# watsonyanghx/GAN_Lib_Tensorflow

Measured on AMD Instinct MI355X. Metric: images/sec (G+D step) SNGAN-ResNet CIFAR-10 bs=64, higher is better.
Workload: dtype bf16; 1 GPU; SNGAN ResNet CIFAR-10 32x32 bs=64 hinge: 1 G update (2x64 fakes) + 5 D updates (64 real + 64 fake) per step; global_batch=64, per_gpu_batch=64, parallelism=dp1, graphs=True, finite=True, collectives_in_graphs=False, grad_wire=fp32

## Files before the change

gan_lib_tensorflow_amd/SNGAN/gan_cifar_resnet.py:

```python
import contextlib
import math
import sys

import numpy as np
import torch
import torch.distributed as _dist

from .. import functional as Fn
from .. import graphs
from .. import kernels as K
from .. import parallel
from ..common import resnet_block as blocks
from ..common.ops import embedding as _embedding
from ..common.ops import linear as _linear
from ..common.ops import conv2d as _conv2d
from ..common.ops import normalization as _normalization
from ..common.ops import sn as _sn
from ..common.ops.sn import NO_OPS
from ..store import ParamStore, get_default_store, set_default_store

BATCH_SIZE = 64
GEN_BS_MULTIPLE = 2
ITERS = 100000
DIM_G = 128
# ... 75 lines not shown
        return 2
    if blocks.FUSE_RES8 and W.dim() == 4 and tuple(W.shape) == (3, 3, 128, 128) and ('D.Block.3.' in name or 'D.Block.4.' in name):
        return 4
    if Fn.IMG16_CONV and name.endswith('D.Block.2.Conv1/Filters') and W.dim() == 4 and W.shape[0] == 3 and W.shape[2] % 64 == 0 and W.shape[3] % 128 == 0 \
            and W.shape[2] % 128 == 0:
        if Fn.FACTOR_LABEL_CONV and LABEL_TABLE and CONDITIONAL and W.shape[2] == 2 * DIM_D:
            return 6
        return 4
    return 0


def _g_prep_kind(name, W):
    if Fn.RES8_CONV and name.endswith(('G.Block.1.Conv1/Filters', 'G.Block.1.Conv2/Filters')) and W.dim() == 4 and W.shape[0] == 3 \
            and W.shape[2] in (128, 256) and W.shape[3] % 128 == 0:
        return 4
    if Fn.PHASE_UPCONV and name.endswith('.Conv1/Filters') and W.dim() == 4 and W.shape[0] == 3:
        return 1
    if Fn.IMG16_CONV and name.endswith('G.Block.2.Conv2/Filters') and W.dim() == 4 and W.shape[0] == 3 and W.shape[2] % 128 == 0 and W.shape[3] % 128 == 0:
        return 4
    return 0


FUSE_SN_TAIL = True
FUSE_FEED = True
LABEL_TABLE = True
FUSED_HEAD = True
HEAD_IN_CHAIN = True


def Discriminator(inputs, labels, update_collection=None, reuse=False, loss_head=None):
# ... 656 lines not shown
```

gan_lib_tensorflow_amd/_lib.py:

```python
import ctypes as C
import os

_HERE = os.path.dirname(os.path.abspath(__file__))
DTYPE = os.environ.get("GANK_DTYPE", "bf16").lower()
if DTYPE not in ("bf16", "fp16"):
    raise RuntimeError(f"GANK_DTYPE={DTYPE!r}: bf16 or fp16")
ACT_DTYPE_NAME = "bfloat16" if DTYPE == "bf16" else "float16"
LIB_PATH = os.path.join(_HERE, os.environ.get("GANK_LIB_NAME", "libgank.so" if DTYPE == "bf16" else "libgank_f16.so"))

P, I, L, F = C.c_void_p, C.c_int, C.c_long, C.c_float

IN_UPSAMPLE2X, IN_RELU, OUT_TANH, DY_UPSAMPLE2X, RES_UPSAMPLE2X, STATS_PREZEROED, OUT_POOLSUM2X = 1, 2, 4, 8, 64, 256, 512
STAT_SLOTS = 16


class SnDesc(C.Structure):
    _fields_ = [(n, P) for n in ("W", "u_in", "u_out", "v", "W_bar", "scal", "a", "b", "bpart",
                                 "dW_bar", "dW", "rowdot", "ga", "u_snap")] + \
               [("K", I), ("C", I), ("row_offset", I), ("chunk_offset", I)]


class WgradItem(C.Structure):
    _fields_ = [("x", P), ("dy", P), ("dw", P), ("dbias", P)]

# ... 51 lines not shown
    "gank_conv2d_general_dgrad": [P, P, P, P, I, I, I, I, I, I, I, I, I, P],
    "gank_conv2d_general_wgrad": [P, P, P, P, I, I, I, I, I, I, I, I, I, I, I, P],
    "gank_res8_chain_fwd": [P, P, P, P, P, P, I, I, I, P],
    "gank_res8_chain_bwd": [P, P, P, P, P, P, P, P, P, I, I, I, P],
    "gank_phase_stack4": [P, P, I, I, I, P],
    "gank_pad_rows": [P, P, C.c_long, I, I, I, I, P],
    "gank_tile_rows": [P, P, I, I, I, P],
    "gank_fewout_pack": [P, P, I, I, I, I, I, P],
    "gank_zero_f32": [P, C.c_long, P],
    "gank_img16_conv3x3": [P, P, P, P, P, P, I, I, I, I, P],
    "gank_cbn_relu_img16_conv3x3": [P, P, P, P, P, P, P, P, P, I, I, I, I, I, I, P, I, P],
    "gank_img16_conv3x3_stats": [P, P, P, P, P, P, I, I, I, I, P, I, P],
    "gank_res8_chain_fwd_head": [P, P, P, P, P, P, P, P, P, I, I, I, P],
    "gank_res8_chain_bwd_head": [C.POINTER(Res8Head), P, P, P, P, P, P, P, I, I, I, P],
    "gank_res8_conv3x3": [P, P, P, P, P, I, I, I, I, P, I, P],
    "gank_im2col_narrow": [P, P, I, I, I, I, I, I, I, I, I, I, P],
    "gank_tap_gather_up2": [P, P, P, I, I, I, I, I, I, I, I, P],
    "gank_tap_scatter_up2": [P, P, I, I, I, I, I, I, I, P],
    "gank_depth_to_space2": [P, P, I, I, I, I, P],
    "gank_space_to_depth2": [P, P, I, I, I, I, P],
    "gank_cpool_res_fprop": [P, P, P, P, P, I, I, I, I, I, I, P],
    "gank_cpool_res_dgrad": [P, P, P, P, I, I, I, I, I, P],
    "gank_cpool_res_dgrad_image_wgrad": [P, P, P, P, P, P, P, P, P, I, I, I, I, I, P, P],
    "gank_sum_slabs": [C.POINTER(SlabJob), I, P],
    "gank_convpool3x3_wgrad_job": [P, P, P, P, P, L, I, I, I, I, I, I, C.POINTER(SlabJob), P],
    "gank_conv2d_wgrad_slab_elems": [I, I, I, I, I, I, I],
    "gank_conv2d_wgrad_slabs": [P, P, P, P, I, I, I, I, I, I, I, F, P, L, C.POINTER(SlabJob), P],
    "gank_conv2d_wgrad_slab_splits": [I, I, I, I, I, I, I],
    "gank_conv2d_wgrad_slabs_rows": [P, P, P, P, I, I, I, I, I, I, I, I, F, P, L, C.POINTER(SlabJob), P],
    "gank_conv2d_wgrad_slabs_rows_tap_sums": [P, P, P, P, I, I, I, I, I, I, I, I, F, P, L, C.POINTER(SlabJob), P, I, P, P],
# ... 158 lines not shown
```

gan_lib_tensorflow_amd/csrc/conv_resident.hip:

```cpp
#include "gank_common.h"
#include "label_conv_dev.h"
#ifdef GANK_TUNING
static __device__ int gank_stats_dbg = 0;
static void gank_stats_dbg_init() {
  static const int v = gank_tune("GANK_STATS_DBG", 0);
  static bool done = false;
  if (!done) { done = true; if (v) (void)hipMemcpyToSymbol(HIP_SYMBOL(gank_stats_dbg), &v, sizeof(int)); }
}
#else
static inline void gank_stats_dbg_init() {}
#endif
#include <stdlib.h>

namespace {
constexpr int RB_C = 128;
constexpr int RB_PPB = RB_C * 2 + 16;
constexpr int RB_RPB = 2944;
constexpr int RB_IMG = 10 * RB_RPB;
constexpr int RB_STEPS = 9 * (RB_C / 16);
constexpr int RB_WBYTES = RB_C * 9 * RB_C * 2;
constexpr int RB_LDS = 2 * RB_IMG;

struct ResFwdArgs {
  const bf16* x;
// ... 2121 lines not shown
  }
  const int grid = N * (Cout / 128);
  if (Cin == 256) {
    constexpr int LDS = G8Geom<256>::IMG > G8_RED_BYTES ? G8Geom<256>::IMG : G8_RED_BYTES;
    GANK_MAX_DYNAMIC_LDS((res8_conv3x3_kernel<256, 12>), LDS, "res8_conv3x3");
    hipLaunchKernelGGL((res8_conv3x3_kernel<256, 12>), dim3(grid), dim3(256), LDS, s, a);
  } else {
    constexpr int LDS = G8Geom<128>::IMG > G8_RED_BYTES ? G8Geom<128>::IMG : G8_RED_BYTES;
    GANK_MAX_DYNAMIC_LDS((res8_conv3x3_kernel<128, 12>), LDS, "res8_conv3x3");
    hipLaunchKernelGGL((res8_conv3x3_kernel<128, 12>), dim3(grid), dim3(256), LDS, s, a);
  }
  gank_prof_end(0, s);
  GANK_LAUNCH_OK("res8_conv3x3");
  return 0;
}
```

gan_lib_tensorflow_amd/csrc/prep_weights.h:

```cpp
#pragma once
#include "gank_common.h"

template <bool SC>
__device__ __forceinline__ float prep_ld(float x, float sg) {
  if constexpr (SC) return x / sg;
  else return x;
}

__device__ __forceinline__ void up_range_R(int a, int i, int& lo, int& hi) {
  if (a == 0) { lo = i == 0 ? 0 : 1; hi = i == 0 ? 0 : 2; } else { lo = i == 0 ? 0 : 2; hi = i == 0 ? 1 : 2; }
}
__device__ __forceinline__ void up_range_S(int u, int& lo, int& hi) {
  lo = u == 0 ? 2 : (u == 1 ? 1 : 0);
  hi = u == 0 ? 2 : (u == 1 ? 2 : (u == 2 ? 1 : 0));
}
template <bool SC = false>
__device__ __forceinline__ float sum_taps(const float* __restrict__ p, long plane, bool flip, int h0, int h1, int w0, int w1, float sg = 1.f) {
  const float mh = h1 > h0 ? 1.f : 0.f, mw = w1 > w0 ? 1.f : 0.f;
  const int t00 = flip ? (2 - h0) * 3 + (2 - w0) : h0 * 3 + w0, t01 = flip ? (2 - h0) * 3 + (2 - w1) : h0 * 3 + w1;
  const int t10 = flip ? (2 - h1) * 3 + (2 - w0) : h1 * 3 + w0, t11 = flip ? (2 - h1) * 3 + (2 - w1) : h1 * 3 + w1;
  const float a = prep_ld<SC>(p[t00 * plane], sg), b = prep_ld<SC>(p[t01 * plane], sg), c = prep_ld<SC>(p[t10 * plane], sg), d = prep_ld<SC>(p[t11 * plane], sg);
  return ((a + mw * b) + mh * c) + (mh * mw) * d;
}

// ... 182 lines not shown
      const int lane = (int)(q & 63);
      long u = q >> 6;
      const int kk = (int)(u % (kc / 16)); u /= (kc / 16);
      const int tap = (int)(u % taps);
      const int rt = (int)(u / taps);
      const int row = rt * 32 + (lane & 31), k0 = kk * 16 + (lane >> 5) * 8;
      bf16x8 o;
#pragma unroll
      for (int j = 0; j < 8; j++) {
        const int k = k0 + j;
        const long cp = d.cin_pitch > 0 ? d.cin_pitch : d.Cin;
        o[j] = f2bf(prep_ld<SC>(isf ? d.w[((long)tap * cp + k) * d.Cout + row] : d.w[((long)(taps - 1 - tap) * cp + row) * d.Cout + k], sg));
      }
      *reinterpret_cast<bf16x8*>(dst + q * 8) = o;
    }
  } else if (d.kind == 5) {
    const bool isf = b < t.nwf[e];
    const long q = (long)(isf ? b : b - t.nwf[e]) * 256 + threadIdx.x;
    const long nchunk = 2L * d.Cin * d.Cout;
    if (q < nchunk) {
      const int lane = (int)(q & 63), r = lane & 31, hh = lane >> 5;
      long u = q >> 6;
      bf16x8 o;
      if (isf) {
        const int kk = (int)(u & 3); u >>= 2;
        const int tap = (int)(u & 15); u >>= 4;
        const int nch = d.Cin >> 6;
        const int chunk = (int)(u % nch), co = (int)(u / nch) * 32 + r;
        int h0, h1, w0, w1;
        up_range_S(tap >> 2, h0, h1);
// ... 76 lines not shown
    }
  }
}


static inline int prep_table_fill(PrepTable& t, const gank_prep_desc* table, int count, int base_index) {
  t = PrepTable{};
  t.count = count;
  int blocks = 0;
  for (int i = 0; i < t.count; i++) {
    const gank_prep_desc& d = table[i];
    const bool ok = d.w && (d.wf || d.wd) && d.ksize >= 1 && d.Cin > 0 && d.Cout > 0;
    if (!ok) { gank_set_error("prep_weights_batched: bad entry %d", base_index + i); return -1; }
    const bool kind_ok = d.kind == 0 || ((d.kind == 1 || d.kind == 2) && d.ksize == 3 && d.wf && d.wd) ||
                         (d.kind == 4 && d.Cin % 32 == 0 && d.Cout % 32 == 0 && (d.cin_pitch == 0 || d.cin_pitch >= d.Cin)) ||
                         (d.kind == 5 && d.ksize == 3 && d.wf && d.wd && d.Cin % 64 == 0 && d.Cout % 32 == 0);
    if (!kind_ok) {
      gank_set_error("prep_weights_batched: entry %d: kind %d needs ksize 3 and both outputs (1, 2, 5) / channels %% 32 == 0 (4) / Cin %% 64 == 0 (5)", base_index + i, d.kind);
      return -1;
    }
    t.d[i] = d;
    const int taps = d.ksize * d.ksize;
    int nwf = d.wf ? (roundup(taps * d.Cin, 64) / 64) * (roundup(d.Cout, 32) / 32) : 0;
    int nwd = d.wd ? cdiv((long)roundup(d.Cin, 32) * roundup(taps * d.Cout, 64), 2048) : 0;
    if (d.kind == 1 || d.kind == 2) {
      t.up[i] = d.kind == 1 ? prep_up_args(1, d.w, d.wf, d.wd, d.Cin, d.Cout) : prep_up_args(2, d.w, d.wd, d.wf, d.Cin, d.Cout);
      const PrepUpSplit sp = prep_up_split(t.up[i], d.kind);
      nwf = sp.ntiles;
      nwd = sp.nelem;
    }
    if (d.kind == 5) nwf = nwd = cdiv(2L * d.Cin * d.Cout, 256);
    if (d.kind == 4) {
      nwf = d.wf ? cdiv((long)d.Cout * taps * d.Cin / 8, 256) : 0;
      nwd = d.wd ? cdiv((long)d.Cin * taps * d.Cout / 8, 256) : 0;
    }
    t.first_block[i] = blocks;
    t.nwf[i] = nwf;
    blocks += nwf + nwd;
  }
  t.first_block[t.count] = blocks;
  return blocks;
}
```

gan_lib_tensorflow_amd/functional.py:

```python
import torch
from torch.autograd import Function

from . import kernels as K

BF16 = K.BF16
POOL_CONV4 = True
CPOOL_RESIDENT = True
PHASE_UPCONV = True
RES8_CONV = True
UPCONV_WGRAD_PHASE = True
IMG16_CONV = True


_boundary_log = None


def boundary(x, tag):
    if _boundary_log is not None and x.requires_grad:
        _boundary_log.append((tag, x))
    return x


class record_boundaries:
    def __enter__(self):
        global _boundary_log
# ... 126 lines not shown
            k, cin, cout = 1, W.shape[0], W.shape[1]
        else:
            k, cin, cout = W.shape[0], W.shape[2], W.shape[3]
        assert x.dim() == 4 and x.shape[3] == cin, (tuple(x.shape), tuple(W.shape))
        assert not (pool_out and (out_tanh or upsample))
        n, h, w, _ = x.shape
        H, Wd = (2 * h, 2 * w) if upsample else (h, w)
        flags = (K.IN_UPSAMPLE2X if upsample else 0) | (K.IN_RELU if in_relu else 0) | (K.OUT_TANH if out_tanh else 0)
        b = bias.detach() if bias is not None else None
        res_up = residual is not None and getattr(residual, "_up2x", False)
        ctx.res_up_orig = res_up
        res8 = (RES8_CONV and k == 3 and not in_relu and not pool_out and not out_tanh and getattr(W, "_prep_res", None) is not None
                and K.res8_conv3x3_ok(n, (H, Wd), cin, cout))
        img16 = (IMG16_CONV and k == 3 and not upsample and not pool_out and not out_tanh
                 and getattr(W, "_prep_res", None) is not None and K.img16_conv3x3_ok(n, (H, Wd), cin, cout))
        phase = upsample and k == 3 and cin % 64 == 0 and not in_relu and PHASE_UPCONV and not res8
        pool4 = pool_out and k == 3 and cin % 64 == 0 and cout % 64 == 0 and POOL_CONV4
        if res_up and (phase or pool_out):
            residual = K.unpool2x2_add(residual, None, 1.0)
            res_up = False
        if res8:
            rflags = (K.IN_UPSAMPLE2X if upsample else 0) | (K.RES_UPSAMPLE2X if res_up else 0)
            if stats_groups:
                y, _Conv2d.last_stats = K.res8_conv3x3(x, W._prep_res[0], b, cout, rflags, residual, stats_groups)
            else:
                y = K.res8_conv3x3(x, W._prep_res[0], b, cout, rflags, residual)
        elif img16:
            iflags = (K.IN_RELU if in_relu else 0) | (K.RES_UPSAMPLE2X if res_up else 0)
            if stats_groups:
                y, _Conv2d.last_stats = K.img16_conv3x3(x, W._prep_res[0], b, cout, iflags, None, residual, stats_groups)
            else:
                y = K.img16_conv3x3(x, W._prep_res[0], b, cout, iflags, None, residual)
        elif phase:
            wph, _ = getattr(W, "_prep_up", None) or K.upconv3x3_prep(W.detach().view(3, 3, cin, cout))
            if stats_groups and not out_tanh:
                y, _Conv2d.last_stats = K.upconv3x3_fprop(x, wph, b, cout, 0, residual, stats_groups)
            else:
                y = K.upconv3x3_fprop(x, wph, b, cout, K.OUT_TANH if out_tanh else 0, residual)
        elif pool4 and getattr(W, "_prep_cpres", None) is not None:
            y = K.cpool_res_fprop(x, W._prep_cpres[0], b, cout, K.IN_RELU if in_relu else 0, residual)
        elif pool4:
            wp4, _ = getattr(W, "_prep_pool", None) or K.convpool3x3_prep(W.detach().view(3, 3, cin, cout))
            y = K.convpool3x3_fprop(x, wp4, b, cout, K.IN_RELU if in_relu else 0, residual)
        elif pool_out:
            wf, _ = _prepared(W, k, cin, cout, True, False)
            yfull = K.conv2d_fprop(x, wf, b, (H, Wd), cout, k, flags)
            y = K.pool2x2(yfull, 0.25, residual)
# ... 7 lines not shown
                if stats_groups and not out_tanh:
                    y, _Conv2d.last_stats = K.conv2d_fprop(x, wf, b, (H, Wd), cout, k, flags | (K.RES_UPSAMPLE2X if res_up else 0), 1.0, residual,
                                                           stats_groups=stats_groups)
                else:
                    y = K.conv2d_fprop(x, wf, b, (H, Wd), cout, k, flags | (K.RES_UPSAMPLE2X if res_up else 0), 1.0, residual)
        ctx.res_up = res_up
        ctx.add_link = ctx.res_link = None
        link = getattr(x, "_add_link", None)
        if link is not None and ctx.needs_input_grad[0] and not (upsample or pool_out or phase or pool4 or res8):
            link.armed = True
            ctx.add_link = link
        rlink = getattr(residual, "_grad_link", None) if residual is not None else None
        if rlink is not None and rlink.armed and not res_up and not ctx.res_up_orig:
            ctx.res_link = rlink
        ctx.save_for_backward(x, W, y if out_tanh else None)
        ctx.cfg = (k, cin, cout, H, Wd, upsample, in_relu, pool_out, out_tanh, bias, phase, pool4)
        if FUSE_IMAGE_WGRAD and x.is_cuda:
            if (k == 3 and cin == 3 and residual is None and not (upsample or in_relu or pool_out or out_tanh or stats_groups)
                    and ctx.needs_input_grad[1] and not ctx.needs_input_grad[0]):
                ctx.sink = _Conv2d.last_sink = ImageWgradSink(x, W, bias)
                ctx.set_materialize_grads(False)
            elif (pool4 and in_relu and getattr(W, "_prep_cpres", None) is not None and ctx.needs_input_grad[0]
                  and getattr(x, "_image_wgrad_sink", None) is not None and K.cpool_res_dgrad_image_wgrad_ok(y, cin)):
                ctx.isink = x._image_wgrad_sink
                ctx.ssink = getattr(residual, "_shortcut_sink", None) if (residual is not None and not ctx.res_up_orig) else None
        ctx.res8 = res8 and W._prep_res[1] is not None and K.res8_conv3x3_ok(n, (8, 8), cout, cin)
        ctx.img16 = img16 and W._prep_res[1] is not None and K.img16_conv3x3_ok(n, (16, 16), cout, cin)
        return y

    @staticmethod
    def backward(ctx, dy):
# ... 35 lines not shown
            elif (CONV1X1_BWD_ONE_LAUNCH and k == 1 and wflags == 0 and scale == 1.0 and ctx.needs_input_grad[0] and ctx.add_link is None
                  and not ctx.img16 and not ctx.res8 and not phase
                  and int(K.lib().gank_conv2d_wgrad_slab_elems(x.shape[0], H, Wd, cin, cout, 1, 0)) == 0
                  and K.conv1x1_wgrad_dgrad_ok(x.shape[0], (H, Wd), cin, cout, _prepared(W, k, cin, cout, False, True)[1])):
                dx_fused = K.conv1x1_wgrad_dgrad(x, g, tgt, _prepared(W, k, cin, cout, False, True)[1], dbias=btgt)
            else:
                K.conv2d_wgrad(x, g, tgt, (H, Wd), k, wflags, scale, dbias=btgt,
                               slab_jobs=_slab_jobs if (SLAB_WGRADS and BATCH_SMALL_WGRADS) else None)
            dW = None if acc else tgt
        elif btgt is not None:
            K.colsum(g, btgt, 1.0)
        if dx_fused is not None:
            dx = dx_fused
        elif ctx.needs_input_grad[0] and ctx.res8:
            dx = K.res8_conv3x3(g, W._prep_res[1], None, cin, K.OUT_POOLSUM2X if upsample else 0)
        elif ctx.needs_input_grad[0] and phase:
            prep = getattr(W, "_prep_up", None) or K.upconv3x3_prep(W.detach().view(3, 3, cin, cout))
            dx = K.upconv3x3_dgrad(g, prep[1], cin)
        elif ctx.needs_input_grad[0] and pool4 and getattr(W, "_prep_cpres", None) is not None and ctx.isink is not None:
            isink, ssink = ctx.isink, ctx.ssink
            t1, _, b1, _ = isink.targets()
            ts = bs_ = xp = None
            if ssink is not None:
                ts, _, bs_, _ = ssink.targets()
                xp = ssink.x
            K.cpool_res_dgrad_image_wgrad(g, W._prep_cpres[1], x, isink.x, t1, b1, xp, ts, bs_,
                                          slab_jobs=_slab_jobs if (SLAB_WGRADS and BATCH_SMALL_WGRADS) else None)
            isink.done = True
            if ssink is not None:
                ssink.done = True
# ... 409 lines not shown
        if self.opt is not None:
            self.opt.pending_sn = None
        return self

    def __exit__(self, *exc):
        global SN_DEFER_APPLY
        SN_DEFER_APPLY = self.prev
        return False


def spectral_norm_batch(Ws, us, snapshot=False, inplace=False, prep=None, label=None, state=None):
    batch = K.SnBatch(list(Ws), [u.detach() for u in us], snapshot, inplace, state=state)
    batch.prep, batch.label = prep, label
    outs = _SpectralNorm.apply(batch, *Ws)
    for o, wb in zip(outs, batch.W_bar):
        for attr in ("_prep", "_prep_up", "_prep_pool", "_prep_res", "_prep_cpres", "_label_T"):
            val = getattr(wb, attr, None)
            if val is not None and o is not wb:
                setattr(o, attr, val)
    return outs, batch


CBN_REMASK = True


class _CondBatchNorm(Function):
    @staticmethod
    def forward(ctx, x, labels, gamma, beta, groups, relu):
        cs = getattr(x, "_cbn_stats", None)
        if cs is not None and cs.groups == groups and cs.sums.shape[-1] == x.shape[-1]:
            y, stats = K.cbn_fwd_from_sums(x, labels, gamma.detach(), beta.detach(), cs, relu)
# ... 843 lines not shown
```

gan_lib_tensorflow_amd/kernels.py:

```python
import ctypes as C

import torch

from . import _lib
from ._lib import IN_UPSAMPLE2X, IN_RELU, OUT_TANH, DY_UPSAMPLE2X, RES_UPSAMPLE2X, STATS_PREZEROED, OUT_POOLSUM2X, SnDesc, PrepDesc, WgradItem, LabelDenseDesc, Res8Head, SlabJob

BF16, F32, I32 = getattr(torch, _lib.ACT_DTYPE_NAME), torch.float32, torch.int32


def _stream():
    return C.c_void_p(torch.cuda.current_stream().cuda_stream)


def _p(t, dtype=None, name="tensor"):
    if t is None:
        return None
    if not t.is_cuda:
        raise RuntimeError(f"gank: {name} must live on the GPU (no CPU path exists)")
    if not t.is_contiguous():
        raise RuntimeError(f"gank: {name} must be contiguous, got strides {t.stride()} for {tuple(t.shape)}")
    if dtype is not None and t.dtype != dtype:
        raise RuntimeError(f"gank: {name} must be {dtype}, got {t.dtype}")
    return C.c_void_p(t.data_ptr())

# ... 3 lines not shown


def lib():
    return _lib.load()


def prep_weights(w, want_f=True, want_d=False):
    k, _, cin, cout = w.shape
    taps = k * k
    wf = torch.empty((_roundup(cout, 32), _roundup(taps * cin, 64)), dtype=BF16, device=w.device) if want_f else None
    wd = torch.empty((_roundup(cin, 32), _roundup(taps * cout, 64)), dtype=BF16, device=w.device) if want_d else None
    _lib.check(lib().gank_conv2d_prep_weights(_p(w, F32, "w"), _p(wf), _p(wd), k, cin, cout, _stream()), "prep_weights")
    return wf, wd


_PREP_ATTR = ("_prep", "_prep_up", "_prep_pool", None, "_prep_res", "_prep_cpres", "_prep_feat")


def _prep_plan(ws, want_d=True, kinds=None, sources=None):
    kinds = list(kinds) if kinds is not None else [0] * len(ws)
    todo = [i for i, kd in enumerate(kinds) if kd is not None]
    table = (PrepDesc * max(len(todo), 1))()
    outs = []
    for slot, i in enumerate(todo):
        w, kind = ws[i], kinds[i]
        if w.dim() == 2:
            k, cin, cout = 1, w.shape[0], w.shape[1]
        else:
            k, cin, cout = w.shape[0], w.shape[2], w.shape[3]
        taps = k * k
        dev = w.device
# ... 13 lines not shown
            wf, wd = getattr(w, "_prep_pool", None) or (torch.empty((_roundup(cout, 32), _roundup(16 * cin, 64)), dtype=BF16, device=dev),
                                                       torch.empty((4, _roundup(cin, 32), 4 * cout), dtype=BF16, device=dev))
        elif kind == 4:
            assert k == 3 and cin % 32 == 0 and cout % 32 == 0
            wf, wd = getattr(w, "_prep_res", None) or (torch.empty(taps * cin * cout, dtype=BF16, device=dev),
                                                      torch.empty(taps * cin * cout, dtype=BF16, device=dev) if want_d else None)
        elif kind == 5:
            assert k == 3 and cin % 64 == 0 and cout % 32 == 0
            wf, wd = getattr(w, "_prep_cpres", None) or (torch.empty(16 * cin * cout, dtype=BF16, device=dev),
                                                        torch.empty(16 * cin * cout, dtype=BF16, device=dev))
        elif kind == 6:
            assert k == 3 and cin % 64 == 0 and cout % 32 == 0
            half = cin // 2
            wf, wd = getattr(w, "_prep_feat", None) or (torch.empty(taps * half * cout, dtype=BF16, device=dev),
                                                       torch.empty(taps * half * cout, dtype=BF16, device=dev) if want_d else None)
        else:
            raise ValueError(f"unknown preparation kind {kind}")
        src = w if sources is None else sources[i]
        d = table[slot]
        d.w, d.wf, d.wd = _p(src.detach(), F32, "w").value, wf.data_ptr(), (wd.data_ptr() if wd is not None else None)
        d.ksize, d.Cin, d.Cout, d.kind = k, cin, cout, kind
        if kind == 6:
            d.Cin, d.kind, d.cin_pitch = cin // 2, 4, cin
        outs.append((wf, wd))
    return table, todo, outs


def _prep_attach(ws, kinds, todo, outs):
    for i, o in zip(todo, outs):
        setattr(ws[i], _PREP_ATTR[kinds[i]], o)
# ... 464 lines not shown
    return y


def res8_conv3x3(x, rf, bias, cout, flags=0, residual=None, stats_groups=0):
    n, cin = x.shape[0], x.shape[3]
    hw = 4 if flags & OUT_POOLSUM2X else 8
    y = torch.empty((n, hw, hw, cout), dtype=BF16, device=x.device)
    if stats_groups:
        sums, pre = stats_arena.take((stats_groups, _lib.STAT_SLOTS, 2, cout), x.device)
        _lib.check(lib().gank_res8_conv3x3(_p(x, BF16, "x"), _p(rf, BF16, "rf"), _p(bias, F32, "bias"), _p(residual, BF16, "residual"), _p(y),
                                           n, cin, cout, flags | (STATS_PREZEROED if pre else 0), _p(sums), stats_groups, _stream()), "res8_conv3x3")
        return y, ConvStats(sums, bias, stats_groups)
    _lib.check(lib().gank_res8_conv3x3(_p(x, BF16, "x"), _p(rf, BF16, "rf"), _p(bias, F32, "bias"), _p(residual, BF16, "residual"), _p(y),
                                       n, cin, cout, flags, None, 0, _stream()), "res8_conv3x3")
    return y


def cpool_res_fprop(x, rf, bias, cout, flags=0, residual=None):
    n, h, w, cin = x.shape
    y = torch.empty((n, h // 2, w // 2, cout), dtype=BF16, device=x.device)
    _lib.check(lib().gank_cpool_res_fprop(_p(x, BF16, "x"), _p(rf, BF16, "rf"), _p(bias, F32, "bias"), _p(residual, BF16, "residual"),
                                          _p(y), n, h // 2, w // 2, cin, cout, flags, _stream()), "cpool_res_fprop")
    return y


def cpool_res_dgrad(dy, rd, cin, relu_ref=None):
    n, hp, wp, cout = dy.shape
    dx = torch.empty((n, 2 * hp, 2 * wp, cin), dtype=BF16, device=dy.device)
    _lib.check(lib().gank_cpool_res_dgrad(_p(dy, BF16, "dy"), _p(rd, BF16, "rd"), _p(relu_ref, BF16, "relu_ref"), _p(dx),
                                          n, hp, wp, cin, cout, _stream()), "cpool_res_dgrad")
# ... 1224 lines not shown
```

include/gank.h:

```cpp
#ifndef GANK_H
#define GANK_H

#include <stddef.h>
#include <stdint.h>

#ifdef __cplusplus
extern "C" {
#endif

#define GANK_VERSION 100

#define GANK_IN_UPSAMPLE2X 1
#define GANK_IN_RELU 2
#define GANK_OUT_TANH 4
#define GANK_DY_UPSAMPLE2X 8
#define GANK_STAT_SLOTS 16
#define GANK_STATS_PREZEROED 256
#define GANK_RES_UPSAMPLE2X 64
#define GANK_OUT_POOLSUM2X 512

int gank_version(void);
int gank_act_dtype(void);
const char* gank_last_error(void);

// ... 84 lines not shown
                             int nblocks, void* stream);
int gank_res8_chain_bwd_head(const gank_res8_head* head, const void* ylast, void* dy_out, const void* const* wd_rfrag,
                             const void* const* h1, const void* const* xin, void* const* g1, void* const* dx, int N, int C,
                             int nblocks, void* stream);

int gank_img16_conv3x3(const void* x, const void* w_rfrag, const float* bias, const void* relu_ref, const void* residual, void* y,
                       int N, int Cin, int Cout, int flags, void* stream);
int gank_cbn_relu_img16_conv3x3(const void* x, const int32_t* labels, const float* gamma, const float* beta, const float* stats,
                                const void* w_rfrag, const float* bias, const void* residual, void* y, int N, int Cin, int Cout,
                                int groups, int n_labels, int flags, float* stat_sums, int stat_groups, void* stream);
int gank_img16_conv3x3_stats(const void* x, const void* w_rfrag, const float* bias, const void* relu_ref, const void* residual, void* y,
                             int N, int Cin, int Cout, int flags, float* stat_sums, int stat_groups, void* stream);

int gank_res8_conv3x3(const void* x, const void* w_rfrag, const float* bias, const void* residual, void* y, int N, int Cin,
                      int Cout, int flags, float* stat_sums, int stat_groups, void* stream);

int gank_cpool_res_fprop(const void* x, const void* w_rfrag, const float* bias, const void* residual, void* y, int N, int Hp,
                         int Wp, int Cin, int Cout, int flags, void* stream);
int gank_cpool_res_dgrad(const void* dy, const void* w_rfrag, const void* relu_ref, void* dx, int N, int Hp, int Wp, int Cin,
                         int Cout, void* stream);
int gank_cpool_res_dgrad_image_wgrad(const void* dy, const void* w_rfrag, const void* relu_ref, const void* x_image, float* dw1,
                                     float* db1, const void* x_pooled, float* dws, float* dbs, int N, int Hp, int Wp, int Cin,
                                     int Cout, float* slabs, void* stream);

int gank_upconv3x3_prep_weights(const float* w, void* wph, void* wd4, int Cin, int Cout, void* stream);
int gank_upconv3x3_fprop(const void* x, const void* wph, const float* bias, const void* residual, void* y,
                         int N, int Hl, int Wl, int Cin, int Cout, int flags, void* stream);
int gank_upconv3x3_fprop_stats(const void* x, const void* wph, const float* bias, const void* residual, void* y,
                               int N, int Hl, int Wl, int Cin, int Cout, int flags, float* stat_sums, int groups, int* produced,
                               void* stream);
// ... 289 lines not shown
```

scratch/seq_dump.py:

```python
import csv, glob, re, sys
f = glob.glob(sys.argv[1] + '/**/*kernel_trace.csv', recursive=True)[0]
rows = sorted(csv.DictReader(open(f)), key=lambda r: int(r['Start_Timestamp']))
n = int(sys.argv[2])
rows = rows[len(rows) // 2:len(rows) // 2 + n]
prev = None
for r in rows:
    s, e = int(r['Start_Timestamp']), int(r['End_Timestamp'])
    name = re.sub(r'\(.*', '', r['Kernel_Name'])
    name = re.sub(r'^void ', '', name)[:60]
    gap = (s - prev) / 1e3 if prev else 0.0
    print(f"{(e - s) / 1e3:8.1f} us  gap {gap:6.1f}  grid {r.get('Grid_Size_X', r.get('Grid_Size', '?')):>8} wg {r.get('Workgroup_Size_X', r.get('Workgroup_Size', '?')):>4}  {name}")
    prev = e
```

Measured before the change: 58320 images/sec.

## Add LDS-resident phase-decomposed upconv kernels for generator block 2 conv1

Adds a resident-image upsample-conv kernel for 8x8 to 16x16 generator convolutions. It decomposes the 2x nearest upsample plus 3x3 conv into four 2x2 phase convolutions. Each block keeps a whole padded 8x8 image in LDS and streams weights through a register ring, and a matching dgrad kernel handles the backward path. A new weight-prep kind 7 produces the phase-summed filters, and the kernel fuses bias, residual and batch-norm statistics. The aim is to replace the general phase-upconv path with fewer launches and better on-chip reuse, at the cost of extra weight-prep work and new specialized code.

```diff
diff --git a/gan_lib_tensorflow_amd/SNGAN/gan_cifar_resnet.py b/gan_lib_tensorflow_amd/SNGAN/gan_cifar_resnet.py
--- a/gan_lib_tensorflow_amd/SNGAN/gan_cifar_resnet.py
+++ b/gan_lib_tensorflow_amd/SNGAN/gan_cifar_resnet.py
@@ -113,6 +113,9 @@
     if Fn.RES8_CONV and name.endswith(('G.Block.1.Conv1/Filters', 'G.Block.1.Conv2/Filters')) and W.dim() == 4 and W.shape[0] == 3 \
             and W.shape[2] in (128, 256) and W.shape[3] % 128 == 0:
         return 4
+    if Fn.RES8_UPCONV and name.endswith('G.Block.2.Conv1/Filters') and W.dim() == 4 and W.shape[0] == 3 \
+            and W.shape[2] in (128, 256) and W.shape[3] in (128, 256):
+        return 7
     if Fn.PHASE_UPCONV and name.endswith('.Conv1/Filters') and W.dim() == 4 and W.shape[0] == 3:
         return 1
     if Fn.IMG16_CONV and name.endswith('G.Block.2.Conv2/Filters') and W.dim() == 4 and W.shape[0] == 3 and W.shape[2] % 128 == 0 and W.shape[3] % 128 == 0:
diff --git a/gan_lib_tensorflow_amd/_lib.py b/gan_lib_tensorflow_amd/_lib.py
--- a/gan_lib_tensorflow_amd/_lib.py
+++ b/gan_lib_tensorflow_amd/_lib.py
@@ -89,6 +89,8 @@
     "gank_res8_chain_fwd_head": [P, P, P, P, P, P, P, P, P, I, I, I, P],
     "gank_res8_chain_bwd_head": [C.POINTER(Res8Head), P, P, P, P, P, P, P, I, I, I, P],
     "gank_res8_conv3x3": [P, P, P, P, P, I, I, I, I, P, I, P],
+    "gank_res8_upconv3x3": [P, P, P, P, P, I, I, I, I, P, I, P],
+    "gank_res8_upconv3x3_dgrad": [P, P, P, P, I, I, I, P],
     "gank_im2col_narrow": [P, P, I, I, I, I, I, I, I, I, I, I, P],
     "gank_tap_gather_up2": [P, P, P, I, I, I, I, I, I, I, I, P],
     "gank_tap_scatter_up2": [P, P, I, I, I, I, I, I, I, P],
diff --git a/gan_lib_tensorflow_amd/csrc/conv_resident.hip b/gan_lib_tensorflow_amd/csrc/conv_resident.hip
--- a/gan_lib_tensorflow_amd/csrc/conv_resident.hip
+++ b/gan_lib_tensorflow_amd/csrc/conv_resident.hip
@@ -2159,3 +2159,303 @@
   GANK_LAUNCH_OK("res8_conv3x3");
   return 0;
 }
+
+namespace {
+constexpr int U8_PF = 16;
+
+struct U8Args {
+  const bf16* x;
+  const bf16* w;
+  const float* bias;
+  const bf16* res;
+  bf16* y;
+  float* stat_sums;
+  int N, Cout, stat_n_per_group;
+  int xcd;
+};
+
+template <int C>
+__device__ __forceinline__ void up8_zero_halo(char* img, int tid) {
+  using G = G8Geom<C>;
+  constexpr int RU = G::RPB / 16, PU = G::PPB / 16;
+  for (int i = tid; i < 2 * RU + 16 * PU; i += 256) {
+    int off;
+    if (i < 2 * RU) off = (i < RU ? 0 : 9 * G::RPB - RU * 16) + i * 16;
+    else {
+      const int j = i - 2 * RU, rr = 1 + j / (2 * PU), k = j % (2 * PU);
+      off = rr * G::RPB + (k < PU ? 0 : 9 * G::PPB - PU * 16) + k * 16;
+    }
+    *reinterpret_cast<u32x4*>(img + off) = u32x4{0u, 0u, 0u, 0u};
+  }
+}
+
+template <int C, int PF, bool FWD>
+__device__ __forceinline__ void up8_phase(f32x16 (&acc)[2], u32x4 (&ring)[PF], const char* smem, int b_base,
+                                          const __amdgpu_buffer_rsrc_t rw, int lane16, int wbase, bool more) {
+  using G = G8Geom<C>;
+  constexpr int NS = 4 * G::KK;
+  static_assert(NS % PF == 0, "the ring position must be the same at the start of every phase");
+  constexpr int PB = 2;
+  u32x4 bq[PB + 1][2];
+  auto read_b = [&](int s, u32x4 (&dst)[2]) {
+    const int tap = s / G::KK, kk = s % G::KK, ta = tap >> 1, tb = tap & 1;
+    const int off = (FWD ? ta : 1 - ta) * G::RPB + (FWD ? tb : 1 - tb) * G::PPB + kk * 32;
+#pragma unroll
+    for (int t = 0; t < 2; t++) dst[t] = *reinterpret_cast<const u32x4*>(smem + b_base + 4 * t * G::RPB + off);
+  };
+#pragma unroll
+  for (int s = 0; s < PB; s++) read_b(s, bq[s]);
+#pragma unroll
+  for (int s = 0; s < NS; s++) {
+    if (s + PB < NS) read_b(s + PB, bq[(s + PB) % (PB + 1)]);
+    const bf16x8 fa = __builtin_bit_cast(bf16x8, ring[s % PF]);
+    __builtin_amdgcn_sched_barrier(0);
+#pragma unroll
+    for (int t = 0; t < 2; t++) acc[t] = GANK_MFMA32(fa, __builtin_bit_cast(bf16x8, bq[s % (PB + 1)][t]), acc[t]);
+    __builtin_amdgcn_sched_barrier(0);
+    if (s + PF < NS || more) ring[s % PF] = __builtin_amdgcn_raw_buffer_load_b128(rw, lane16, wbase + (s + PF) * 1024, 0);
+    __builtin_amdgcn_sched_barrier(0);
+  }
+}
+
+template <int C, int PF>
+__global__ __launch_bounds__(256) void res8_upconv3x3_kernel(U8Args a) {
+  using G = G8Geom<C>;
+  constexpr int NT = 256, U = C / 8, NS = 4 * G::KK;
+  extern __shared__ __attribute__((aligned(16))) char smem[];
+  const int tid = threadIdx.x, lane = tid & 63;
+  const int ct = __builtin_amdgcn_readfirstlane(tid >> 6);
+  const int r = lane & 31, h = lane >> 5;
+  const int ntc = a.Cout >> 7;
+  const int lid = a.xcd ? xcd_remap(blockIdx.x, gridDim.x) : blockIdx.x;
+  const int n = lid / ntc, half = lid - n * ntc;
+  const int co0 = half * 128 + ct * 32;
+  const int b_base = (r >> 3) * G::RPB + (r & 7) * G::PPB + h * 16;
+  const int wtile = (half * 4 + ct) * 4 * NS * 1024;
+  const __amdgpu_buffer_rsrc_t rw = __builtin_amdgcn_make_buffer_rsrc(const_cast<bf16*>(a.w), 0, (a.Cout >> 5) * 4 * NS * 1024, 0x00020000);
+
+  u32x4 ring[PF];
+#pragma unroll
+  for (int s = 0; s < PF; s++) ring[s] = __builtin_amdgcn_raw_buffer_load_b128(rw, lane * 16, wtile + s * 1024, 0);
+
+  up8_zero_halo<C>(smem, tid);
+  {
+    const bf16* src = a.x + (long)n * 64 * C;
+#pragma unroll
+    for (int it = 0; it < 64 * U / NT; it++) {
+      const int q = tid + it * NT, px = q / U, u = q % U;
+      *reinterpret_cast<u32x4*>(smem + ((px >> 3) + 1) * G::RPB + ((px & 7) + 1) * G::PPB + u * 16) =
+          *reinterpret_cast<const u32x4*>(src + px * C + u * 8);
+    }
+  }
+  __syncthreads();
+
+  const bool stats = a.stat_sums != nullptr;
+  float s1[2][8], s2[2][8];
+#pragma unroll
+  for (int q = 0; q < 2; q++)
+#pragma unroll
+    for (int e = 0; e < 8; e++) { s1[q][e] = 0.f; s2[q][e] = 0.f; }
+
+#pragma unroll 1
+  for (int p = 0; p < 4; p++) {
+    const int py = p >> 1, px = p & 1;
+    f32x16 acc[2];
+#pragma unroll
+    for (int t = 0; t < 2; t++)
+#pragma unroll
+      for (int e = 0; e < 16; e++) acc[t][e] = 0.f;
+    up8_phase<C, PF, true>(acc, ring, smem, b_base + py * G::RPB + px * G::PPB, rw, lane * 16, wtile + p * NS * 1024, p < 3);
+
+#pragma unroll
+    for (int t = 0; t < 2; t++) {
+      const long opix = ((long)n * 16 + 2 * (4 * t + (r >> 3)) + py) * 16 + 2 * (r & 7) + px;
+#pragma unroll
+      for (int q = 0; q < 2; q++) {
+        const int c = co0 + 16 * q + 8 * h;
+        float v[8];
+        acc_widen(acc[t], q, 1.0f, v);
+        if (a.res) {
+          const bf16x8 rv = *reinterpret_cast<const bf16x8*>(a.res + opix * a.Cout + c);
+#pragma unroll
+          for (int e = 0; e < 8; e++) v[e] += bf2f(rv[e]);
+        }
+        f32x4 b0 = {0.f, 0.f, 0.f, 0.f}, b1 = {0.f, 0.f, 0.f, 0.f};
+        if (a.bias) { b0 = *reinterpret_cast<const f32x4*>(a.bias + c); b1 = *reinterpret_cast<const f32x4*>(a.bias + c + 4); }
+        bf16x8 o;
+#pragma unroll
+        for (int e = 0; e < 8; e++) {
+          s1[q][e] += v[e];
+          s2[q][e] += v[e] * v[e];
+          o[e] = f2bf(v[e] + (e < 4 ? b0[e] : b1[e - 4]));
+        }
+        *reinterpret_cast<bf16x8*>(a.y + opix * a.Cout + c) = o;
+      }
+    }
+  }
+  if (stats) {
+    __syncthreads();
+    float* red = reinterpret_cast<float*>(smem) + ct * 2048;
+#pragma unroll
+    for (int q = 0; q < 2; q++)
+#pragma unroll
+      for (int e = 0; e < 8; e++) {
+        red[((0 * 2 + q) * 2 + h) * 256 + e * 32 + r] = s1[q][e];
+        red[((1 * 2 + q) * 2 + h) * 256 + e * 32 + r] = s2[q][e];
+      }
+    __builtin_amdgcn_fence(__ATOMIC_RELEASE, "wavefront");
+    __builtin_amdgcn_wave_barrier();
+    __builtin_amdgcn_fence(__ATOMIC_ACQUIRE, "wavefront");
+    const int st = lane >> 5, cw = lane & 31, qq = cw >> 4, hh = (cw >> 3) & 1, ee = cw & 7;
+    const float* src = red + ((st * 2 + qq) * 2 + hh) * 256 + ee * 32;
+    float tsum = 0.f;
+#pragma unroll
+    for (int i = 0; i < 8; i++) {
+      const f32x4 t4 = *reinterpret_cast<const f32x4*>(src + 4 * i);
+      tsum += (t4[0] + t4[1]) + (t4[2] + t4[3]);
+    }
+    float* dst = a.stat_sums + ((long)(n / a.stat_n_per_group) * GANK_STAT_SLOTS + (blockIdx.x % GANK_STAT_SLOTS)) * 2 * a.Cout;
+#ifdef GANK_TUNING
+    if (gank_stats_dbg) return;
+#endif
+    atomicAdd(dst + st * a.Cout + co0 + cw, tsum);
+  }
+}
+
+template <int C, int PF>
+__global__ __launch_bounds__(256) void res8_upconv3x3_dgrad_kernel(U8Args a) {
+  using G = G8Geom<C>;
+  constexpr int NT = 256, U = C / 8, NS = 4 * G::KK, NLD = 64 * U / NT;
+  extern __shared__ __attribute__((aligned(16))) char smem[];
+  const int tid = threadIdx.x, lane = tid & 63;
+  const int ct = __builtin_amdgcn_readfirstlane(tid >> 6);
+  const int r = lane & 31, h = lane >> 5;
+  const int ntc = a.Cout >> 7;
+  const int lid = a.xcd ? xcd_remap(blockIdx.x, gridDim.x) : blockIdx.x;
+  const int n = lid / ntc, half = lid - n * ntc;
+  const int co0 = half * 128 + ct * 32;
+  const int b_base = (r >> 3) * G::RPB + (r & 7) * G::PPB + h * 16;
+  const int wtile = (half * 4 + ct) * 4 * NS * 1024;
+  const __amdgpu_buffer_rsrc_t rw = __builtin_amdgcn_make_buffer_rsrc(const_cast<bf16*>(a.w), 0, (a.Cout >> 5) * 4 * NS * 1024, 0x00020000);
+
+  u32x4 ring[PF];
+#pragma unroll
+  for (int s = 0; s < PF; s++) ring[s] = __builtin_amdgcn_raw_buffer_load_b128(rw, lane * 16, wtile + s * 1024, 0);
+
+  const bf16* src = a.x + (long)n * 256 * C;
+  u32x4 rP[NLD];
+  auto load_phase = [&](int p) {
+#pragma unroll
+    for (int it = 0; it < NLD; it++) {
+      const int q = tid + it * NT, px = q / U, u = q % U;
+      rP[it] = *reinterpret_cast<const u32x4*>(src + ((2 * (px >> 3) + (p >> 1)) * 16 + 2 * (px & 7) + (p & 1)) * C + u * 8);
+    }
+  };
+  load_phase(0);
+  up8_zero_halo<C>(smem, tid);
+
+  f32x16 acc[2];
+#pragma unroll
+  for (int t = 0; t < 2; t++)
+#pragma unroll
+    for (int e = 0; e < 16; e++) acc[t][e] = 0.f;
+
+#pragma unroll 1
+  for (int p = 0; p < 4; p++) {
+    const int py = p >> 1, px = p & 1;
+    if (p > 0) __syncthreads();
+#pragma unroll
+    for (int it = 0; it < NLD; it++) {
+      const int q = tid + it * NT, pp = q / U, u = q % U;
+      *reinterpret_cast<u32x4*>(smem + ((pp >> 3) + 1) * G::RPB + ((pp & 7) + 1) * G::PPB + u * 16) = rP[it];
+    }
+    __syncthreads();
+    if (p < 3) load_phase(p + 1);
+    up8_phase<C, PF, false>(acc, ring, smem, b_base + (1 - py) * G::RPB + (1 - px) * G::PPB, rw, lane * 16, wtile + p * NS * 1024, p < 3);
+  }
+
+#pragma unroll
+  for (int t = 0; t < 2; t++) {
+    const long pix = (long)n * 64 + 32 * t + r;
+#pragma unroll
+    for (int q = 0; q < 2; q++) {
+      const int c = co0 + 16 * q + 8 * h;
+      float v[8];
+      acc_widen(acc[t], q, 1.0f, v);
+      bf16x8 o;
+      if (a.res) {
+        const bf16x8 m = *reinterpret_cast<const bf16x8*>(a.res + pix * a.Cout + c);
+#pragma unroll
+        for (int e = 0; e < 8; e++) o[e] = f2bf(bf2f(m[e]) > 0.f ? v[e] : 0.f);
+      } else {
+#pragma unroll
+        for (int e = 0; e < 8; e++) o[e] = f2bf(v[e]);
+      }
+      *reinterpret_cast<bf16x8*>(a.y + pix * a.Cout + c) = o;
+    }
+  }
+}
+
+template <int C>
+static int up8_launch_fwd(const U8Args& a, hipStream_t s) {
+  constexpr int LDS = G8Geom<C>::IMG > G8_RED_BYTES ? G8Geom<C>::IMG : G8_RED_BYTES;
+  GANK_MAX_DYNAMIC_LDS((res8_upconv3x3_kernel<C, U8_PF>), LDS, "res8_upconv3x3");
+  hipLaunchKernelGGL((res8_upconv3x3_kernel<C, U8_PF>), dim3(a.N * (a.Cout / 128)), dim3(256), LDS, s, a);
+  return 0;
+}
+template <int C>
+static int up8_launch_dgrad(const U8Args& a, hipStream_t s) {
+  constexpr int LDS = G8Geom<C>::IMG;
+  GANK_MAX_DYNAMIC_LDS((res8_upconv3x3_dgrad_kernel<C, U8_PF>), LDS, "res8_upconv3x3_dgrad");
+  hipLaunchKernelGGL((res8_upconv3x3_dgrad_kernel<C, U8_PF>), dim3(a.N * (a.Cout / 128)), dim3(256), LDS, s, a);
+  return 0;
+}
+}
+
+extern "C" int gank_res8_upconv3x3(const void* x, const void* w_rfrag, const float* bias, const void* residual, void* y, int N, int Cin,
+                                   int Cout, int flags, float* stat_sums, int stat_groups, void* stream) {
+  GANK_REQUIRE(x && w_rfrag && y && N > 0, "res8_upconv3x3: null pointer");
+  GANK_REQUIRE((Cin == 256 || Cin == 128) && Cout % 128 == 0, "res8_upconv3x3: built for Cin 128 | 256 and Cout %% 128 == 0 (got %d, %d)", Cin, Cout);
+  GANK_REQUIRE((flags & ~GANK_STATS_PREZEROED) == 0, "res8_upconv3x3: unsupported flags 0x%x", flags & ~GANK_STATS_PREZEROED);
+  GANK_REQUIRE(!stat_sums || (stat_groups > 0 && N % stat_groups == 0), "res8_upconv3x3: batch %d not divisible by %d towers", N, stat_groups);
+  GANK_REQUIRE((long)N * 256 * Cout < (1L << 30) && (long)N * 64 * Cin < (1L << 30), "res8_upconv3x3: tensor too large");
+  U8Args a{};
+  a.x = (const bf16*)x; a.w = (const bf16*)w_rfrag; a.bias = bias; a.res = (const bf16*)residual; a.y = (bf16*)y;
+  a.stat_sums = stat_sums; a.N = N; a.Cout = Cout;
+  a.stat_n_per_group = stat_sums ? N / stat_groups : 1;
+  a.xcd = resident_xcd_env();
+  hipStream_t s = (hipStream_t)stream;
+  gank_prof_begin(0, 2.0 * N * 256.0 * 4.0 * Cin * Cout, s,
+                  2.0 * (N * 64.0 * Cin + 16.0 * Cin * Cout + N * 256.0 * Cout + (residual ? N * 256.0 * Cout : 0.0)));
+  gank_prof_tag(0, Cin == 256 ? "res8_upconv3x3_kernel<256, 16>" : "res8_upconv3x3_kernel<128, 16>");
+  if (stat_sums) gank_stats_dbg_init();
+  if (stat_sums && !(flags & GANK_STATS_PREZEROED)) {
+    const int nz = stat_groups * GANK_STAT_SLOTS * 2 * Cout;
+    hipLaunchKernelGGL(g8_zero_kernel, dim3((nz + 255) / 256), dim3(256), 0, s, stat_sums, nz);
+  }
+  const int rc = Cin == 256 ? up8_launch_fwd<256>(a, s) : up8_launch_fwd<128>(a, s);
+  gank_prof_end(0, s);
+  if (rc) return rc;
+  GANK_LAUNCH_OK("res8_upconv3x3");
+  return 0;
+}
+
+extern "C" int gank_res8_upconv3x3_dgrad(const void* dy, const void* wd_rfrag, const void* relu_ref, void* dx, int N, int Cin, int Cout,
+                                         void* stream) {
+  GANK_REQUIRE(dy && wd_rfrag && dx && N > 0, "res8_upconv3x3_dgrad: null pointer");
+  GANK_REQUIRE((Cout == 256 || Cout == 128) && Cin % 128 == 0, "res8_upconv3x3_dgrad: built for Cout 128 | 256 and Cin %% 128 == 0 (got %d, %d)", Cout, Cin);
+  GANK_REQUIRE((long)N * 256 * Cout < (1L << 30) && (long)N * 64 * Cin < (1L << 30), "res8_upconv3x3_dgrad: tensor too large");
+  U8Args a{};
+  a.x = (const bf16*)dy; a.w = (const bf16*)wd_rfrag; a.res = (const bf16*)relu_ref; a.y = (bf16*)dx;
+  a.N = N; a.Cout = Cin; a.stat_n_per_group = 1;
+  a.xcd = resident_xcd_env();
+  hipStream_t s = (hipStream_t)stream;
+  gank_prof_begin(0, 2.0 * N * 256.0 * 4.0 * Cin * Cout, s,
+                  2.0 * (N * 256.0 * Cout + 16.0 * Cin * Cout + N * 64.0 * Cin + (relu_ref ? N * 64.0 * Cin : 0.0)));
+  gank_prof_tag(0, Cout == 256 ? "res8_upconv3x3_dgrad_kernel<256, 16>" : "res8_upconv3x3_dgrad_kernel<128, 16>");
+  const int rc = Cout == 256 ? up8_launch_dgrad<256>(a, s) : up8_launch_dgrad<128>(a, s);
+  gank_prof_end(0, s);
+  if (rc) return rc;
+  GANK_LAUNCH_OK("res8_upconv3x3_dgrad");
+  return 0;
+}
diff --git a/gan_lib_tensorflow_amd/csrc/prep_weights.h b/gan_lib_tensorflow_amd/csrc/prep_weights.h
--- a/gan_lib_tensorflow_amd/csrc/prep_weights.h
+++ b/gan_lib_tensorflow_amd/csrc/prep_weights.h
@@ -220,6 +220,28 @@
       }
       *reinterpret_cast<bf16x8*>(dst + q * 8) = o;
     }
+  } else if (d.kind == 7) {
+    const bool isf = b < t.nwf[e];
+    const int kc = isf ? d.Cin : d.Cout;
+    const long q = (long)(isf ? b : b - t.nwf[e]) * 256 + threadIdx.x;
+    const long nchunk = 2L * d.Cin * d.Cout;
+    if (q < nchunk) {
+      const int lane = (int)(q & 63);
+      long u = q >> 6;
+      const int kk = (int)(u % (kc / 16)); u /= (kc / 16);
+      const int tap = (int)(u & 3), phase = (int)((u >> 2) & 3);
+      const int row = (int)(u >> 4) * 32 + (lane & 31), k0 = kk * 16 + (lane >> 5) * 8;
+      int h0, h1, w0, w1;
+      up_range_R(phase >> 1, tap >> 1, h0, h1);
+      up_range_R(phase & 1, tap & 1, w0, w1);
+      bf16x8 o;
+#pragma unroll
+      for (int j = 0; j < 8; j++) {
+        const int ci = isf ? k0 + j : row, co = isf ? row : k0 + j;
+        o[j] = f2bf(sum_taps<SC>(d.w + (long)ci * d.Cout + co, (long)d.Cin * d.Cout, false, h0, h1, w0, w1, sg));
+      }
+      *reinterpret_cast<bf16x8*>((bf16*)(isf ? d.wf : d.wd) + q * 8) = o;
+    }
   } else if (d.kind == 5) {
     const bool isf = b < t.nwf[e];
     const long q = (long)(isf ? b : b - t.nwf[e]) * 256 + threadIdx.x;
@@ -326,9 +348,10 @@
     if (!ok) { gank_set_error("prep_weights_batched: bad entry %d", base_index + i); return -1; }
     const bool kind_ok = d.kind == 0 || ((d.kind == 1 || d.kind == 2) && d.ksize == 3 && d.wf && d.wd) ||
                          (d.kind == 4 && d.Cin % 32 == 0 && d.Cout % 32 == 0 && (d.cin_pitch == 0 || d.cin_pitch >= d.Cin)) ||
-                         (d.kind == 5 && d.ksize == 3 && d.wf && d.wd && d.Cin % 64 == 0 && d.Cout % 32 == 0);
+                         (d.kind == 5 && d.ksize == 3 && d.wf && d.wd && d.Cin % 64 == 0 && d.Cout % 32 == 0) ||
+                         (d.kind == 7 && d.ksize == 3 && d.wf && d.wd && d.Cin % 32 == 0 && d.Cout % 32 == 0);
     if (!kind_ok) {
-      gank_set_error("prep_weights_batched: entry %d: kind %d needs ksize 3 and both outputs (1, 2, 5) / channels %% 32 == 0 (4) / Cin %% 64 == 0 (5)", base_index + i, d.kind);
+      gank_set_error("prep_weights_batched: entry %d: kind %d needs ksize 3 and both outputs (1, 2, 5, 7) / channels %% 32 == 0 (4, 7) / Cin %% 64 == 0 (5)", base_index + i, d.kind);
       return -1;
     }
     t.d[i] = d;
@@ -341,7 +364,7 @@
       nwf = sp.ntiles;
       nwd = sp.nelem;
     }
-    if (d.kind == 5) nwf = nwd = cdiv(2L * d.Cin * d.Cout, 256);
+    if (d.kind == 5 || d.kind == 7) nwf = nwd = cdiv(2L * d.Cin * d.Cout, 256);
     if (d.kind == 4) {
       nwf = d.wf ? cdiv((long)d.Cout * taps * d.Cin / 8, 256) : 0;
       nwd = d.wd ? cdiv((long)d.Cin * taps * d.Cout / 8, 256) : 0;
diff --git a/gan_lib_tensorflow_amd/functional.py b/gan_lib_tensorflow_amd/functional.py
--- a/gan_lib_tensorflow_amd/functional.py
+++ b/gan_lib_tensorflow_amd/functional.py
@@ -9,6 +9,7 @@
 PHASE_UPCONV = True
 RES8_CONV = True
 UPCONV_WGRAD_PHASE = True
+RES8_UPCONV = True
 IMG16_CONV = True
 
 
@@ -165,9 +166,11 @@
                 and K.res8_conv3x3_ok(n, (H, Wd), cin, cout))
         img16 = (IMG16_CONV and k == 3 and not upsample and not pool_out and not out_tanh
                  and getattr(W, "_prep_res", None) is not None and K.img16_conv3x3_ok(n, (H, Wd), cin, cout))
-        phase = upsample and k == 3 and cin % 64 == 0 and not in_relu and PHASE_UPCONV and not res8
+        up8 = (RES8_UPCONV and upsample and k == 3 and not in_relu and not out_tanh and not res8
+               and getattr(W, "_prep_upres", None) is not None and K.res8_upconv3x3_ok(n, (H, Wd), cin, cout))
+        phase = upsample and k == 3 and cin % 64 == 0 and not in_relu and PHASE_UPCONV and not res8 and not up8
         pool4 = pool_out and k == 3 and cin % 64 == 0 and cout % 64 == 0 and POOL_CONV4
-        if res_up and (phase or pool_out):
+        if res_up and (phase or pool_out or up8):
             residual = K.unpool2x2_add(residual, None, 1.0)
             res_up = False
         if res8:
@@ -182,6 +185,11 @@
                 y, _Conv2d.last_stats = K.img16_conv3x3(x, W._prep_res[0], b, cout, iflags, None, residual, stats_groups)
             else:
                 y = K.img16_conv3x3(x, W._prep_res[0], b, cout, iflags, None, residual)
+        elif up8:
+            if stats_groups:
+                y, _Conv2d.last_stats = K.res8_upconv3x3(x, W._prep_upres[0], b, cout, residual, stats_groups)
+            else:
+                y = K.res8_upconv3x3(x, W._prep_upres[0], b, cout, residual)
         elif phase:
             wph, _ = getattr(W, "_prep_up", None) or K.upconv3x3_prep(W.detach().view(3, 3, cin, cout))
             if stats_groups and not out_tanh:
@@ -219,7 +227,8 @@
         if rlink is not None and rlink.armed and not res_up and not ctx.res_up_orig:
             ctx.res_link = rlink
         ctx.save_for_backward(x, W, y if out_tanh else None)
-        ctx.cfg = (k, cin, cout, H, Wd, upsample, in_relu, pool_out, out_tanh, bias, phase, pool4)
+        ctx.up8 = up8 and K.res8_upconv3x3_ok(n, (H, Wd), cout, cin)
+        ctx.cfg = (k, cin, cout, H, Wd, upsample, in_relu, pool_out, out_tanh, bias, phase or (up8 and PHASE_UPCONV and cin % 64 == 0), pool4)
         if FUSE_IMAGE_WGRAD and x.is_cuda:
             if (k == 3 and cin == 3 and residual is None and not (upsample or in_relu or pool_out or out_tanh or stats_groups)
                     and ctx.needs_input_grad[1] and not ctx.needs_input_grad[0]):
@@ -285,6 +294,8 @@
             dx = dx_fused
         elif ctx.needs_input_grad[0] and ctx.res8:
             dx = K.res8_conv3x3(g, W._prep_res[1], None, cin, K.OUT_POOLSUM2X if upsample else 0)
+        elif ctx.needs_input_grad[0] and ctx.up8:
+            dx = K.res8_upconv3x3_dgrad(g, W._prep_upres[1], cin)
         elif ctx.needs_input_grad[0] and phase:
             prep = getattr(W, "_prep_up", None) or K.upconv3x3_prep(W.detach().view(3, 3, cin, cout))
             dx = K.upconv3x3_dgrad(g, prep[1], cin)
@@ -724,7 +735,7 @@
     batch.prep, batch.label = prep, label
     outs = _SpectralNorm.apply(batch, *Ws)
     for o, wb in zip(outs, batch.W_bar):
-        for attr in ("_prep", "_prep_up", "_prep_pool", "_prep_res", "_prep_cpres", "_label_T"):
+        for attr in ("_prep", "_prep_up", "_prep_pool", "_prep_res", "_prep_cpres", "_prep_upres", "_label_T"):
             val = getattr(wb, attr, None)
             if val is not None and o is not wb:
                 setattr(o, attr, val)
diff --git a/gan_lib_tensorflow_amd/kernels.py b/gan_lib_tensorflow_amd/kernels.py
--- a/gan_lib_tensorflow_amd/kernels.py
+++ b/gan_lib_tensorflow_amd/kernels.py
@@ -41,7 +41,7 @@
     return wf, wd
 
 
-_PREP_ATTR = ("_prep", "_prep_up", "_prep_pool", None, "_prep_res", "_prep_cpres", "_prep_feat")
+_PREP_ATTR = ("_prep", "_prep_up", "_prep_pool", None, "_prep_res", "_prep_cpres", "_prep_feat", "_prep_upres")
 
 
 def _prep_plan(ws, want_d=True, kinds=None, sources=None):
@@ -85,6 +85,10 @@
             half = cin // 2
             wf, wd = getattr(w, "_prep_feat", None) or (torch.empty(taps * half * cout, dtype=BF16, device=dev),
                                                        torch.empty(taps * half * cout, dtype=BF16, device=dev) if want_d else None)
+        elif kind == 7:
+            assert k == 3 and cin % 32 == 0 and cout % 32 == 0
+            wf, wd = getattr(w, "_prep_upres", None) or (torch.empty(16 * cin * cout, dtype=BF16, device=dev),
+                                                        torch.empty(16 * cin * cout, dtype=BF16, device=dev))
         else:
             raise ValueError(f"unknown preparation kind {kind}")
         src = w if sources is None else sources[i]
@@ -579,6 +583,33 @@
     _lib.check(lib().gank_res8_conv3x3(_p(x, BF16, "x"), _p(rf, BF16, "rf"), _p(bias, F32, "bias"), _p(residual, BF16, "residual"), _p(y),
                                        n, cin, cout, flags, None, 0, _stream()), "res8_conv3x3")
     return y
+
+
+def res8_upconv3x3_ok(n, hw, cin, cout):
+    return tuple(hw) == (16, 16) and cin in (128, 256) and cout % 128 == 0 and n * 256 * max(cin, cout) < (1 << 30)
+
+
+def res8_upconv3x3(x, rf, bias, cout, residual=None, stats_groups=0):
+    n, cin = x.shape[0], x.shape[3]
+    assert tuple(x.shape[1:3]) == (8, 8), x.shape
+    y = torch.empty((n, 16, 16, cout), dtype=BF16, device=x.device)
+    if stats_groups:
+        sums, pre = stats_arena.take((stats_groups, _lib.STAT_SLOTS, 2, cout), x.device)
+        _lib.check(lib().gank_res8_upconv3x3(_p(x, BF16, "x"), _p(rf, BF16, "rf"), _p(bias, F32, "bias"), _p(residual, BF16, "residual"), _p(y),
+                                             n, cin, cout, STATS_PREZEROED if pre else 0, _p(sums), stats_groups, _stream()), "res8_upconv3x3")
+        return y, ConvStats(sums, bias, stats_groups)
+    _lib.check(lib().gank_res8_upconv3x3(_p(x, BF16, "x"), _p(rf, BF16, "rf"), _p(bias, F32, "bias"), _p(residual, BF16, "residual"), _p(y),
+                                         n, cin, cout, 0, None, 0, _stream()), "res8_upconv3x3")
+    return y
+
+
+def res8_upconv3x3_dgrad(dy, rd, cin, relu_ref=None):
+    n, cout = dy.shape[0], dy.shape[3]
+    assert tuple(dy.shape[1:3]) == (16, 16), dy.shape
+    dx = torch.empty((n, 8, 8, cin), dtype=BF16, device=dy.device)
+    _lib.check(lib().gank_res8_upconv3x3_dgrad(_p(dy, BF16, "dy"), _p(rd, BF16, "rd"), _p(relu_ref, BF16, "relu_ref"), _p(dx),
+                                               n, cin, cout, _stream()), "res8_upconv3x3_dgrad")
+    return dx
 
 
 def cpool_res_fprop(x, rf, bias, cout, flags=0, residual=None):
diff --git a/include/gank.h b/include/gank.h
--- a/include/gank.h
+++ b/include/gank.h
@@ -122,6 +122,11 @@
 
 int gank_res8_conv3x3(const void* x, const void* w_rfrag, const float* bias, const void* residual, void* y, int N, int Cin,
                       int Cout, int flags, float* stat_sums, int stat_groups, void* stream);
+
+int gank_res8_upconv3x3(const void* x, const void* w_rfrag, const float* bias, const void* residual, void* y, int N, int Cin,
+                        int Cout, int flags, float* stat_sums, int stat_groups, void* stream);
+int gank_res8_upconv3x3_dgrad(const void* dy, const void* wd_rfrag, const void* relu_ref, void* dx, int N, int Cin, int Cout,
+                              void* stream);
 
 int gank_cpool_res_fprop(const void* x, const void* w_rfrag, const float* bias, const void* residual, void* y, int N, int Hp,
                          int Wp, int Cin, int Cout, int flags, void* stream);
diff --git a/scratch/seq_dump.py b/scratch/seq_dump.py
--- a/scratch/seq_dump.py
+++ b/scratch/seq_dump.py
@@ -6,7 +6,7 @@
 prev = None
 for r in rows:
     s, e = int(r['Start_Timestamp']), int(r['End_Timestamp'])
-    name = re.sub(r'\(.*', '', r['Kernel_Name'])
+    name = re.sub(r'\(.*', '', r['Kernel_Name'].replace('(anonymous namespace)::', ''))
     name = re.sub(r'^void ', '', name)[:60]
     gap = (s - prev) / 1e3 if prev else 0.0
     print(f"{(e - s) / 1e3:8.1f} us  gap {gap:6.1f}  grid {r.get('Grid_Size_X', r.get('Grid_Size', '?')):>8} wg {r.get('Workgroup_Size_X', r.get('Workgroup_Size', '?')):>4}  {name}")
```

Result: no change. 58520 images/sec, median of 6 (+0.3%).
